# utiasDSL/gym-pybullet-drones

Hardware: AMD Instinct MI355X
Metric: env steps/sec (whole node), HoverAviary N=65536 drones @240Hz (higher is better)
Workload: dtype f32

## Files before the change

gym_pybullet_drones_amd/csrc/gpd_common.inc:

```
#pragma once
#include <hip/hip_runtime.h>
#include <rccl/rccl.h>
#include <dlfcn.h>

#include <cstdio>
#include <cstdlib>
#include <cstring>
#include <string>
#include <type_traits>

#include "gpd.h"

namespace {

#pragma clang fp contract(off)

#ifndef GPD_BLOCK
#define GPD_BLOCK 256
#endif
constexpr int kBlock = GPD_BLOCK;

template <auto V> using Const = std::integral_constant<decltype(V), V>;

}
// ... 88 lines not shown
    return (stride0 < 0 || stride1 < 0 || stride2 < 0) ? bad(GPD_EINVAL, "strides must be non-negative") : 0;
}
[[maybe_unused]] int check_ranges(Refuse bad, const GpdStepCfg* cfg) {
    if (cfg->act_type < GPD_ACT_RPM || cfg->act_type > GPD_ACT_DIRECT_RPM) return bad(GPD_EINVAL, "unknown act_type");
    return (cfg->task < GPD_TASK_NONE || cfg->task > GPD_TASK_MULTIHOVER) ? bad(GPD_EINVAL, "unknown task") : 0;
}
[[maybe_unused]] int check_positive(Refuse bad, const GpdStepCfg* cfg) {
    const bool ok = cfg->num_envs > 0 && cfg->drones_per_env > 0 && cfg->substeps > 0;
    return ok ? 0 : bad(GPD_EINVAL, "num_envs, drones_per_env and substeps must be positive");
}
[[maybe_unused]] int check_flags(Refuse bad, const GpdStepCfg* cfg) { return (cfg->physics_flags & ~31u) ? bad(GPD_EINVAL, "unknown physics flag") : 0; }
[[maybe_unused]] int check_extent(Refuse bad, int64_t N, int64_t ld, const char* pitch = "state.ld") {
    if (ld < N) return bad(GPD_EINVAL, pitch, " < num_envs*drones_per_env");
    return N > (1LL << 26) ? bad(GPD_ERANGE, "more than 2^26 drones per launch (32-bit byte offsets)") : 0;
}
[[maybe_unused]] int check_needs(Refuse bad, const GpdParams* params, const GpdState* state, const GpdStepCfg* cfg, const float* target_pos,
                                 const float* init_pose) {
    const bool pid = cfg->act_type == GPD_ACT_PID || cfg->act_type == GPD_ACT_VEL || cfg->act_type == GPD_ACT_ONE_D_PID;
    if (pid && state && !state->pid) return bad(GPD_EINVAL, "PID action type needs state.pid");
    if (pid && params->pid_kf <= 0.0f) return bad(GPD_ENOTSUP, "no DSLPID controller for this airframe (CF2X/CF2P only)");
    if ((cfg->physics_flags & GPD_PHYS_DRAG) && state && !state->last_rpm) return bad(GPD_EINVAL, "GPD_PHYS_DRAG needs state.last_rpm");
    if (cfg->task != GPD_TASK_NONE && !target_pos) return bad(GPD_EINVAL, "task needs target_pos");
    return (cfg->auto_reset && !init_pose) ? bad(GPD_EINVAL, "auto_reset needs init_pose") : 0;
}
[[maybe_unused]] void dummy_target(GpdStepCfg& c, const float*& target_pos, const float* readable) {
    if (c.task == GPD_TASK_NONE) { target_pos = readable; c.target_per_env = 0; }
}
template <class F>
auto with_ext_plant(bool ext, bool plant, F&& f) {
    if (plant) return ext ? f(Const<true>{}, Const<true>{}) : f(Const<false>{}, Const<true>{});
    return ext ? f(Const<true>{}, Const<false>{}) : f(Const<false>{}, Const<false>{});
}

struct Mat3 {
    float r00, r01, r02, r10, r11, r12, r20, r21, r22;
    float m22;
};

__device__ __forceinline__ float fast_rcp(float x) { return __builtin_amdgcn_rcpf(x); }
__device__ __forceinline__ float fast_sqrt(float x) { return __builtin_amdgcn_sqrtf(x); }
__device__ __forceinline__ float fast_rsq(float x) { return __builtin_amdgcn_rsqf(x); }
__device__ __forceinline__ float fast_exp(float x) { return __builtin_amdgcn_exp2f(x * 1.44269504088896340736f); }

typedef float fp2 __attribute__((ext_vector_type(2)));
__device__ __forceinline__ fp2 fma2(fp2 a, fp2 b, fp2 c) { return __builtin_elementwise_fma(a, b, c); }
__device__ __forceinline__ fp2 splat(float s) { return fp2{s, s}; }

__device__ __forceinline__ uint64_t lane_mask_opaque(bool p) {
    uint64_t m = __builtin_amdgcn_ballot_w64(p);
    asm volatile("" : "+s"(m));
    return m;
}
#define any_lane(p) __builtin_expect(lane_mask_opaque(p) != 0, 0)


__device__ __forceinline__ float atan2_poly(float y, float x) {
#pragma clang fp contract(off)
    const float ax = fabsf(x), ay = fabsf(y);
    const float mx = fmaxf(ax, ay), mn = fminf(ax, ay);
    float t = mn * fast_rcp(mx);
    t = (mx == 0.0f) ? 0.0f : t;
    const float u = t * t;
    float p = 2.766283504e-03f;
    p = fmaf(p, u, -1.573124913e-02f);
    p = fmaf(p, u, 4.213762361e-02f);
    p = fmaf(p, u, -7.456854827e-02f);
    p = fmaf(p, u, 1.061837064e-01f);
    p = fmaf(p, u, -1.419779779e-01f);
    p = fmaf(p, u, 1.999187203e-01f);
    p = fmaf(p, u, -3.333303671e-01f);
    p = fmaf(p, u, 9.999999818e-01f);
    p *= t;
    p = (ay > ax) ? (1.57079632679489661923f - p) : p;
    p = (x < 0.0f) ? (3.14159265358979323846f - p) : p;
    return copysignf(p, y);
}

__device__ __forceinline__ fp2 atan2_poly2(fp2 y, fp2 x) {
#pragma clang fp contract(off)
    const float ax0 = fabsf(x.x), ay0 = fabsf(y.x), ax1 = fabsf(x.y), ay1 = fabsf(y.y);
    const float mx0 = fmaxf(ax0, ay0), mn0 = fminf(ax0, ay0), mx1 = fmaxf(ax1, ay1), mn1 = fminf(ax1, ay1);
    fp2 t = fp2{mn0, mn1} * fp2{fast_rcp(mx0), fast_rcp(mx1)};
    t = fp2{(mx0 == 0.0f) ? 0.0f : t.x, (mx1 == 0.0f) ? 0.0f : t.y};
    const fp2 u = t * t;
    fp2 p = splat(2.766283504e-03f);
    p = fma2(p, u, splat(-1.573124913e-02f));
    p = fma2(p, u, splat(4.213762361e-02f));
    p = fma2(p, u, splat(-7.456854827e-02f));
    p = fma2(p, u, splat(1.061837064e-01f));
    p = fma2(p, u, splat(-1.419779779e-01f));
    p = fma2(p, u, splat(1.999187203e-01f));
    p = fma2(p, u, splat(-3.333303671e-01f));
    p = fma2(p, u, splat(9.999999818e-01f));
    p = p * t;
    float p0 = p.x, p1 = p.y;
    p0 = (ay0 > ax0) ? (1.57079632679489661923f - p0) : p0;
    p1 = (ay1 > ax1) ? (1.57079632679489661923f - p1) : p1;
    p0 = (x.x < 0.0f) ? (3.14159265358979323846f - p0) : p0;
    p1 = (x.y < 0.0f) ? (3.14159265358979323846f - p1) : p1;
    return fp2{copysignf(p0, y.x), copysignf(p1, y.y)};
}

__device__ __forceinline__ float asin_poly(float s) {
#pragma clang fp contract(off)
    return atan2_poly(s, fast_sqrt(fmaxf((1.0f - s) * (1.0f + s), 0.0f)));
}

__device__ __forceinline__ Mat3 quat_to_mat(float x, float y, float z, float w) {
    const float d = fmaf(x, x, fmaf(y, y, fmaf(z, z, w * w)));
    const float s = 2.0f * fast_rcp(d);
    const fp2 xys = fp2{x, y} * splat(s);
    const float xs = xys.x, ys = xys.y, zs = z * s;
    const fp2 wxy = splat(w) * xys;
    const float wx = wxy.x, wy = wxy.y, wz = w * zs;
    Mat3 R;
    R.r00 = 1.0f - fmaf(y, ys, z * zs); R.r01 = fmaf(x, ys, -wz);           R.r02 = fmaf(x, zs, wy);
    R.r10 = fmaf(x, ys, wz);            R.r11 = 1.0f - fmaf(x, xs, z * zs); R.r12 = fmaf(y, zs, -wx);
    R.m22 = fmaf(x, xs, y * ys);
    R.r20 = fmaf(x, zs, -wy);           R.r21 = fmaf(y, zs, wx);            R.r22 = 1.0f - R.m22;
    return R;
}

__device__ __forceinline__ void quat_to_rpy(float x, float y, float z, float w,
                                            float& roll, float& pitch, float& yaw) {
#pragma clang fp contract(off)
    const float sarg = -2.0f * fmaf(x, z, -(w * y));
    const float ww_zz = fmaf(w, w, z * z);
    const float xx_yy = fmaf(x, x, y * y);
    const float ww_yy = fmaf(w, w, -(y * y));
    const float xx_zz = fmaf(x, x, -(z * z));
    const fp2 ry = atan2_poly2(splat(2.0f) * fp2{fmaf(y, z, w * x), fmaf(x, y, w * z)}, fp2{ww_zz - xx_yy, ww_yy + xx_zz});
    roll = ry.x;
    pitch = asin_poly(fminf(fmaxf(sarg, -1.0f), 1.0f));
    yaw = ry.y;
    const bool gimbal = fabsf(sarg) >= 0.99999f;
    if (any_lane(gimbal)) {
        asm volatile("; gimbal lock: rare");
        if (gimbal) {
            const bool neg = sarg < 0.0f;
            roll = 0.0f;
            pitch = neg ? -1.57079632679489661923f : 1.57079632679489661923f;
            yaw = 2.0f * (neg ? atan2_poly(x, -y) : atan2_poly(-x, y));
        }
    }
}

__device__ __forceinline__ float clampf(float v, float lo, float hi) {
    return fminf(fmaxf(v, lo), hi);
}

struct Kin {
    float px, py, pz, qx, qy, qz, qw, vx, vy, vz, wx, wy, wz;
};

struct Pid {
    float ipx, ipy, ipz, lr, lp, ly, irx, iry, irz;
};

__device__ __forceinline__ void dslpid(const GpdParams& P, float dt, float inv_dt, const Kin& k, float roll, float pitch,
                                       float yaw, const Mat3& R, float tx, float ty, float tz, float tyaw,
                                       float tvx, float tvy, float tvz, float trr, float trp, float try_,
                                       Pid& s, float rpm[4], float pos_e[3], float* yaw_e) {
    const float epx = tx - k.px, epy = ty - k.py, epz = tz - k.pz;
    const float evx = tvx - k.vx, evy = tvy - k.vy, evz = tvz - k.vz;
    s.ipx = clampf(fmaf(epx, dt, s.ipx), -2.0f, 2.0f);
    s.ipy = clampf(fmaf(epy, dt, s.ipy), -2.0f, 2.0f);
    s.ipz = clampf(clampf(fmaf(epz, dt, s.ipz), -2.0f, 2.0f), -0.15f, 0.15f);
    const float fx = fmaf(P.d_for[0], evx, fmaf(P.i_for[0], s.ipx, P.p_for[0] * epx));
    const float fy = fmaf(P.d_for[1], evy, fmaf(P.i_for[1], s.ipy, P.p_for[1] * epy));
    const float fz = fmaf(P.d_for[2], evz, fmaf(P.i_for[2], s.ipz, P.p_for[2] * epz)) + P.pid_gravity;
    const float along = fmaxf(0.0f, fmaf(fz, R.r22, fmaf(fy, R.r12, fx * R.r02)));
    const float base_pwm = (fast_sqrt(along * P.pid_inv_4kf) - P.pwm2rpm_const) * P.inv_pwm2rpm_scale;
    const float fn = fast_rsq(fmaf(fz, fz, fmaf(fy, fy, fx * fx)));
    const float zbx = fx * fn, zby = fy * fn, zbz = fz * fn;
    float sy, cy;
    sincosf(tyaw, &sy, &cy);
    float ybx = -(zbz * sy);
    float yby = zbz * cy;
    float ybz = fmaf(zbx, sy, -(zby * cy));
    const float yn = fast_rsq(fmaf(ybz, ybz, fmaf(yby, yby, ybx * ybx)));
    ybx *= yn; yby *= yn; ybz *= yn;
    const float xbx = fmaf(yby, zbz, -(ybz * zby));
    const float xby = fmaf(ybz, zbx, -(ybx * zbz));
    const float xbz = fmaf(ybx, zby, -(yby * zbx));
    const float m21 = fmaf(zbz, R.r21, fmaf(zby, R.r11, zbx * R.r01)), m12 = fmaf(ybz, R.r22, fmaf(yby, R.r12, ybx * R.r02));
    const float m02 = fmaf(xbz, R.r22, fmaf(xby, R.r12, xbx * R.r02)), m20 = fmaf(zbz, R.r20, fmaf(zby, R.r10, zbx * R.r00));
    const float m10 = fmaf(ybz, R.r20, fmaf(yby, R.r10, ybx * R.r00)), m01 = fmaf(xbz, R.r21, fmaf(xby, R.r11, xbx * R.r01));
    const float erx = m21 - m12, ery = m02 - m20, erz = m10 - m01;
    const float ewx = fmaf(-(roll - s.lr), inv_dt, trr);
    const float ewy = fmaf(-(pitch - s.lp), inv_dt, trp);
    const float ewz = fmaf(-(yaw - s.ly), inv_dt, try_);
    s.lr = roll; s.lp = pitch; s.ly = yaw;
    s.irx = clampf(clampf(fmaf(-erx, dt, s.irx), -1500.0f, 1500.0f), -1.0f, 1.0f);
    s.iry = clampf(clampf(fmaf(-ery, dt, s.iry), -1500.0f, 1500.0f), -1.0f, 1.0f);
    s.irz = clampf(fmaf(-erz, dt, s.irz), -1500.0f, 1500.0f);
    const float t0 = clampf(fmaf(P.i_tor[0], s.irx, fmaf(P.d_tor[0], ewx, -(P.p_tor[0] * erx))), -3200.0f, 3200.0f);
    const float t1 = clampf(fmaf(P.i_tor[1], s.iry, fmaf(P.d_tor[1], ewy, -(P.p_tor[1] * ery))), -3200.0f, 3200.0f);
    const float t2 = clampf(fmaf(P.i_tor[2], s.irz, fmaf(P.d_tor[2], ewz, -(P.p_tor[2] * erz))), -3200.0f, 3200.0f);
#pragma unroll
    for (int m = 0; m < 4; ++m) {
        const float pwm = clampf(fmaf(P.mixer[3 * m + 2], t2, fmaf(P.mixer[3 * m + 1], t1, fmaf(P.mixer[3 * m], t0, base_pwm))),
                                 P.min_pwm, P.max_pwm);
        rpm[m] = fmaf(P.pwm2rpm_scale, pwm, P.pwm2rpm_const);
    }
    if (pos_e) { pos_e[0] = epx; pos_e[1] = epy; pos_e[2] = epz; }
    if (yaw_e) {
        *yaw_e = atan2_poly(-ybx, xbx) - yaw;
    }
}

__device__ __forceinline__ float thrust_dev(const GpdParams& P, float rpm) {
    return fmaf(P.KF * (rpm - P.hover_rpm), rpm + P.hover_rpm, P.hover_resid);
}
__device__ __forceinline__ float thrust_dev_norm(const GpdParams& P, float e) {
    return P.hover_thrust * (e * (2.0f + e));
}
__device__ __forceinline__ fp2 thrust_dev_norm2(const GpdParams& P, fp2 e) {
    return splat(P.hover_thrust) * (e * (splat(2.0f) + e));
}

struct PlantParams : GpdParams {
    float norm_thrust;
    float norm_gap;
};
__device__ __forceinline__ float thrust_dev_norm(const PlantParams& P, float e) {
    return P.norm_thrust * (e * (2.0f + e)) - P.norm_gap;
}
__device__ __forceinline__ fp2 thrust_dev_norm2(const PlantParams& P, fp2 e) {
    return splat(P.norm_thrust) * (e * (splat(2.0f) + e)) - splat(P.norm_gap);
}

template <bool EXT, bool AV = true>
__device__ __forceinline__ void substep(const GpdParams& P, float h, uint32_t flags, const float g[4],
                                        float drag_rpm_sum, float dw_force, Kin& k,
                                        float& avx, float& avy, float& avz) {
    const Mat3 R = quat_to_mat(k.qx, k.qy, k.qz, k.qw);
    float f0 = g[0], f1 = g[1], f2 = g[2], f3 = g[3];
    if (EXT && (flags & GPD_PHYS_GND)) {
        float e[4];
#pragma unroll
        for (int i = 0; i < 4; i += 2) {
            fp2 hz = fma2(splat(R.r21), fp2{P.prop_y[i], P.prop_y[i + 1]}, fma2(splat(R.r20), fp2{P.prop_x[i], P.prop_x[i + 1]}, splat(k.pz)));
            hz = fp2{fmaxf(hz.x, P.gnd_eff_h_clip), fmaxf(hz.y, P.gnd_eff_h_clip)};
            const fp2 ratio = splat(0.25f * P.prop_radius) * fp2{fast_rcp(hz.x), fast_rcp(hz.y)};
            const fp2 ei = ((splat(P.hover_thrust) + fp2{g[i], g[i + 1]}) * splat(P.gnd_eff_coeff)) * (ratio * ratio);
            e[i] = ei.x; e[i + 1] = ei.y;
        }
        const float sarg = -2.0f * fmaf(k.qx, k.qz, -(k.qw * k.qy));
        const float a = 2.0f * fmaf(k.qy, k.qz, k.qw * k.qx);
        const float b = fmaf(k.qw, k.qw, k.qz * k.qz) - fmaf(k.qx, k.qx, k.qy * k.qy);
        const bool on = (sarg > -0.99999f) && (sarg < 0.99999f) && (b > 0.0f || (a == 0.0f && b == 0.0f));
        if (on) { f0 += e[0]; f1 += e[1]; f2 += e[2]; f3 += e[3]; }
    }
    float dev = ((f0 + f1) + f2) + f3;
    if (EXT && (flags & GPD_PHYS_DW)) dev += dw_force;
    const float T = P.GRAVITY + dev;
    const fp2 Fxy = fp2{R.r02, R.r12} * splat(T);
    float Fx = Fxy.x, Fy = Fxy.y, Fz = fmaf(R.r22, dev, -(P.GRAVITY * R.m22));
    if (EXT && (flags & GPD_PHYS_DRAG)) {
        const float wsum = drag_rpm_sum * (6.28318530717958647692f / 60.0f);
        Fx = fmaf(-(P.drag_coeff[0] * k.vx), wsum, Fx);
        Fy = fmaf(-(P.drag_coeff[1] * k.vy), wsum, Fy);
        Fz = fmaf(-(P.drag_coeff[2] * k.vz), wsum, Fz);
    }
    if (EXT && (flags & GPD_PHYS_DAMP)) {
        const float vn = fast_sqrt(fmaf(k.vz, k.vz, fmaf(k.vy, k.vy, k.vx * k.vx)));
        const float ml = -(P.M * GPD_BULLET_DAMPING) * (1.0f + vn);
        Fx = fmaf(ml, k.vx, Fx); Fy = fmaf(ml, k.vy, Fy); Fz = fmaf(ml, k.vz, Fz);
    }
    const float kz = (P.drone_model == GPD_MODEL_RACE) ? -P.km_over_kf : P.km_over_kf;
    const float tz = kz * (((-g[0] + g[1]) - g[2]) + g[3]);
    const float arm = P.L * 0.70710678118654752440f;
    const float arm_x = (P.drone_model == GPD_MODEL_CF2X) ? -arm : arm;
    const float tx_x = (((f0 + f1) - f2) - f3) * arm_x, ty_x = (((-f0 + f1) + f2) - f3) * arm;
    const float tx_p = (f1 - f3) * P.L, ty_p = (-f0 + f2) * P.L;
    const uint32_t plus = (P.drone_model == GPD_MODEL_CF2P) ? 0xffffffffu : 0u;
    float tx = __uint_as_float((__float_as_uint(tx_p) & plus) | (__float_as_uint(tx_x) & ~plus));
    float ty = __uint_as_float((__float_as_uint(ty_p) & plus) | (__float_as_uint(ty_x) & ~plus));
    const fp2 jwxy = fp2{P.J[0], P.J[1]} * fp2{k.wx, k.wy};
    const float jwx = jwxy.x, jwy = jwxy.y, jwz = P.J[2] * k.wz;
    fp2 txy = fp2{tx, ty} - fp2{fmaf(k.wy, jwz, -(k.wz * jwy)), fmaf(k.wz, jwx, -(k.wx * jwz))};
    float tzz = tz - fmaf(k.wx, jwy, -(k.wy * jwx));
    if (EXT && (flags & GPD_PHYS_DAMP)) {
        const float wn = fast_sqrt(fmaf(k.wz, k.wz, fmaf(k.wy, k.wy, k.wx * k.wx)));
        const float da = -GPD_BULLET_DAMPING * (1.0f + wn);
        txy = fma2(jwxy, splat(da), txy);
        tzz = fmaf(jwz, da, tzz);
    }
    const fp2 hh = splat(h);
    const fp2 vxy = fma2(hh, fp2{Fx, Fy} * splat(P.inv_M), fp2{k.vx, k.vy});
    k.vx = vxy.x; k.vy = vxy.y; k.vz = fmaf(h, Fz * P.inv_M, k.vz);
    const fp2 wxy = fma2(hh, fp2{P.J_INV[0], P.J_INV[1]} * txy, fp2{k.wx, k.wy});
    k.wx = wxy.x; k.wy = wxy.y; k.wz = fmaf(h, P.J_INV[2] * tzz, k.wz);
    const fp2 pxy = fma2(hh, vxy, fp2{k.px, k.py});
    k.px = pxy.x; k.py = pxy.y; k.pz = fmaf(h, k.vz, k.pz);
    if (EXT && (flags & GPD_PHYS_GROUND)) {
        const bool hit = (k.pz < P.ground_z) | ((k.pz <= P.ground_z) & (k.vz < 0.0f));
        k.pz = hit ? P.ground_z : k.pz;
        k.vz = hit ? fmaxf(k.vz, 0.0f) : k.vz;
        k.vx = hit ? 0.0f : k.vx;
        k.vy = hit ? 0.0f : k.vy;
    }
    const float n2 = fmaf(k.wz, k.wz, fmaf(k.wy, k.wy, k.wx * k.wx));
    const float u = n2 * (0.25f * h * h);
    const fp2 uu = splat(u);
    const fp2 csp = fma2(fma2(fma2(fma2(fp2{2.412107309e-05f, 2.693749890e-06f}, uu, fp2{-1.388295778e-03f, -1.983586443e-04f}), uu,
                                  fp2{4.166645522e-02f, 8.333314057e-03f}), uu, fp2{-4.999999736e-01f, -1.666666643e-01f}), uu,
                        fp2{9.999999995e-01f, 1.0f});
    float cs = csp.x;
    float sc = csp.y * (0.5f * h);
    const bool tumbling = !(u <= 1.0f);
    if (any_lane(tumbling)) {
        asm volatile("; tumbling: rare");
        if (tumbling) {
            const float n = sqrtf(n2);
            float sn;
            sincosf(n * h * 0.5f, &sn, &cs);
            sc = sn / n;
        }
    }
    {
        const float lx = fmaf(k.wx, k.qw, fmaf(k.wz, k.qy, -(k.wy * k.qz)));
        const float ly = fmaf(k.wy, k.qw, fmaf(k.wx, k.qz, -(k.wz * k.qx)));
        const float lz = fmaf(k.wz, k.qw, fmaf(k.wy, k.qx, -(k.wx * k.qy)));
        const float lw = -fmaf(k.wz, k.qz, fmaf(k.wy, k.qy, k.wx * k.qx));
        const bool turn = n2 > 1e-16f;
        const fp2 nxy = fma2(splat(sc), fp2{lx, ly}, splat(cs) * fp2{k.qx, k.qy});
        const fp2 nzw = fma2(splat(sc), fp2{lz, lw}, splat(cs) * fp2{k.qz, k.qw});
        k.qx = turn ? nxy.x : k.qx; k.qy = turn ? nxy.y : k.qy;
        k.qz = turn ? nzw.x : k.qz; k.qw = turn ? nzw.y : k.qw;
    }
    if (AV) {
        const fp2 axy = fma2(fp2{R.r02, R.r12}, splat(k.wz), fma2(fp2{R.r01, R.r11}, splat(k.wy), fp2{R.r00, R.r10} * splat(k.wx)));
        avx = axy.x; avy = axy.y;
        avz = fmaf(R.r22, k.wz, fmaf(R.r21, k.wy, R.r20 * k.wx));
    }
}

__device__ __forceinline__ float ld_row(const float* __restrict__ base, int64_t ld, int r, uint32_t off4) {
    return *reinterpret_cast<const float*>(reinterpret_cast<const char*>(base + r * ld) + off4);
}
template <bool PLANT> using plant_t = std::conditional_t<PLANT, PlantParams, const GpdParams&>;
template <bool PLANT>
__device__ __forceinline__ plant_t<PLANT> plant_of(const GpdParams& P, const float* __restrict__ rows, int64_t ld, uint32_t off4) {
    if constexpr (PLANT) {
        PlantParams Q;
        static_cast<GpdParams&>(Q) = P;
        Q.M = ld_row(rows, ld, GPD_PLANT_M, off4);
        Q.inv_M = ld_row(rows, ld, GPD_PLANT_INV_M, off4);
        Q.KF = ld_row(rows, ld, GPD_PLANT_KF, off4);
        Q.GRAVITY = ld_row(rows, ld, GPD_PLANT_GRAVITY, off4);
        Q.J[0] = ld_row(rows, ld, GPD_PLANT_J, off4);
        Q.J[1] = ld_row(rows, ld, GPD_PLANT_J + 1, off4);
        Q.J[2] = ld_row(rows, ld, GPD_PLANT_J + 2, off4);
        Q.J_INV[0] = ld_row(rows, ld, GPD_PLANT_J_INV, off4);
        Q.J_INV[1] = ld_row(rows, ld, GPD_PLANT_J_INV + 1, off4);
        Q.J_INV[2] = ld_row(rows, ld, GPD_PLANT_J_INV + 2, off4);
        Q.km_over_kf = ld_row(rows, ld, GPD_PLANT_KM_OVER_KF, off4);
        Q.gnd_eff_coeff = ld_row(rows, ld, GPD_PLANT_GND_EFF, off4);
        Q.drag_coeff[0] = ld_row(rows, ld, GPD_PLANT_DRAG, off4);
        Q.drag_coeff[1] = ld_row(rows, ld, GPD_PLANT_DRAG + 1, off4);
        Q.drag_coeff[2] = ld_row(rows, ld, GPD_PLANT_DRAG + 2, off4);
        Q.hover_thrust = ld_row(rows, ld, GPD_PLANT_HOVER_THRUST, off4);
        Q.hover_resid = ld_row(rows, ld, GPD_PLANT_HOVER_RESID, off4);
        Q.norm_thrust = ld_row(rows, ld, GPD_PLANT_NORM_THRUST, off4);
        Q.norm_gap = ld_row(rows, ld, GPD_PLANT_NORM_GAP, off4);
        return Q;
    } else {
        (void)rows; (void)ld; (void)off4;
        return P;
    }
}
template <bool PLANT>
__device__ __forceinline__ void plant_live(const plant_t<PLANT>& Q) {
    if constexpr (PLANT)
        asm volatile("" :: "v"(Q.M), "v"(Q.inv_M), "v"(Q.KF), "v"(Q.GRAVITY), "v"(Q.J[0]), "v"(Q.J[1]), "v"(Q.J[2]), "v"(Q.J_INV[0]),
                           "v"(Q.J_INV[1]), "v"(Q.J_INV[2]), "v"(Q.km_over_kf), "v"(Q.gnd_eff_coeff), "v"(Q.drag_coeff[0]),
                           "v"(Q.drag_coeff[1]), "v"(Q.drag_coeff[2]), "v"(Q.hover_thrust), "v"(Q.hover_resid), "v"(Q.norm_thrust),
                           "v"(Q.norm_gap) : "memory");
    else
        (void)Q;
}

template <bool NT = false>
__device__ __forceinline__ void st_row(float* __restrict__ base, int64_t ld, int r, uint32_t off4, float v) {
    float* p = reinterpret_cast<float*>(reinterpret_cast<char*>(base + r * ld) + off4);
    if (NT) __builtin_nontemporal_store(v, p);
    else *p = v;
}

__device__ __forceinline__ const float4* kin_P(const float* kin, int64_t ld) { (void)ld; return reinterpret_cast<const float4*>(kin); }
__device__ __forceinline__ const float4* kin_Q(const float* kin, int64_t ld) { return reinterpret_cast<const float4*>(kin + 4 * ld); }
__device__ __forceinline__ const float4* kin_V(const float* kin, int64_t ld) { return reinterpret_cast<const float4*>(kin + 8 * ld); }
__device__ __forceinline__ float4* kin_P(float* kin, int64_t ld) { (void)ld; return reinterpret_cast<float4*>(kin); }
__device__ __forceinline__ float4* kin_Q(float* kin, int64_t ld) { return reinterpret_cast<float4*>(kin + 4 * ld); }
__device__ __forceinline__ float4* kin_V(float* kin, int64_t ld) { return reinterpret_cast<float4*>(kin + 8 * ld); }

__device__ __forceinline__ void store_obs12(float* __restrict__ obs, uint32_t n, float px, float py, float pz,
                                            float roll, float pitch, float yaw, float vx, float vy, float vz,
                                            float ax, float ay, float az) {
    float4* o = reinterpret_cast<float4*>(reinterpret_cast<char*>(obs) + n * 48u);
    o[0] = make_float4(px, py, pz, roll);
    o[1] = make_float4(pitch, yaw, vx, vy);
    o[2] = make_float4(vz, ax, ay, az);
}

__device__ __forceinline__ void wg_barrier() {
    __builtin_amdgcn_s_waitcnt(0xC07F);
    __builtin_amdgcn_s_barrier();
}

struct Lane {
    uint32_t n;
    uint32_t env;
    int tid;
    int le, d;
    int base;
    bool active;
    bool shfl;
};

struct Carry {
    Kin k;
    Pid s;
    float l0, l1, l2, l3;
    int counter;
    float dw_in;
    float roll, pitch, yaw;
};

struct StepOut {
    float o[12];
    float to[12];
    float rew;
    bool term, trunc, reset;
};

template <bool PID, int AW, int ACT, class PP>
__device__ __forceinline__ void map_action(const PP& P, const GpdStepCfg& C, const float4 act, Carry& c,
                                           float rpm[4], float g[4]) {
    const Kin& k = c.k;
    const int act_type = ACT >= 0 ? ACT : C.act_type;
    rpm[0] = rpm[1] = rpm[2] = rpm[3] = 0.0f;
    if (!PID) {
        if (AW == 1) {
            const float e = 0.05f * act.x;
            rpm[0] = rpm[1] = rpm[2] = rpm[3] = fmaf(P.hover_rpm, e, P.hover_rpm);
            g[0] = g[1] = g[2] = g[3] = thrust_dev_norm(P, e);
        } else if (act_type == GPD_ACT_RPM) {
            const fp2 e01 = splat(0.05f) * fp2{act.x, act.y}, e23 = splat(0.05f) * fp2{act.z, act.w};
            const fp2 r01 = fma2(splat(P.hover_rpm), e01, splat(P.hover_rpm)), r23 = fma2(splat(P.hover_rpm), e23, splat(P.hover_rpm));
            const fp2 g01 = thrust_dev_norm2(P, e01), g23 = thrust_dev_norm2(P, e23);
            rpm[0] = r01.x; rpm[1] = r01.y; rpm[2] = r23.x; rpm[3] = r23.y;
            g[0] = g01.x; g[1] = g01.y; g[2] = g23.x; g[3] = g23.y;
        } else {
            const bool clip = act_type == GPD_ACT_RAW_RPM;
            const float lo = clip ? 0.0f : -3.0e38f, hi = clip ? P.max_rpm : 3.0e38f;
            rpm[0] = clampf(act.x, lo, hi); rpm[1] = clampf(act.y, lo, hi);
            rpm[2] = clampf(act.z, lo, hi); rpm[3] = clampf(act.w, lo, hi);
#pragma unroll
            for (int i = 0; i < 4; ++i) g[i] = thrust_dev(P, rpm[i]);
        }
    } else {
        float tx = k.px, ty = k.py, tz = k.pz, tyaw = 0.0f, tvx = 0.0f, tvy = 0.0f, tvz = 0.0f;
        if (AW == 3) {
            const float dx = act.x - k.px, dy = act.y - k.py, dz = act.z - k.pz;
            const float d2 = fmaf(dz, dz, fmaf(dy, dy, dx * dx));
            if (fast_sqrt(d2) <= 1.0f) { tx = act.x; ty = act.y; tz = act.z; }
            else { const float id = fast_rsq(d2); tx = fmaf(dx, id, k.px); ty = fmaf(dy, id, k.py); tz = fmaf(dz, id, k.pz); }
        } else if (AW == 4) {
            const float nn2 = fmaf(act.z, act.z, fmaf(act.y, act.y, act.x * act.x));
            const float sp = P.speed_limit * fabsf(act.w);
            if (nn2 != 0.0f) { const float in = fast_rsq(nn2); tvx = sp * (act.x * in); tvy = sp * (act.y * in); tvz = sp * (act.z * in); }
            tyaw = c.yaw;
        } else {
            tz = fmaf(0.1f, act.x, k.pz);
        }
        const Mat3 R = quat_to_mat(k.qx, k.qy, k.qz, k.qw);
        dslpid(P, C.ctrl_dt, C.inv_ctrl_dt, k, c.roll, c.pitch, c.yaw, R, tx, ty, tz, tyaw, tvx, tvy, tvz, 0.0f, 0.0f, 0.0f,
               c.s, rpm, nullptr, nullptr);
#pragma unroll
        for (int i = 0; i < 4; ++i) g[i] = thrust_dev(P, rpm[i]);
    }
}

__device__ __forceinline__ void task_single(const GpdStepCfg& C, float px, float py, float pz, float roll, float pitch,
                                            int counter, float tgx, float tgy, float tgz, float& rew, bool& term,
                                            bool& trunc) {
    const fp2 exy = fp2{tgx, tgy} - fp2{px, py};
    const float ex = exy.x, ey = exy.y, ez = tgz - pz;
    const float my_dist = fast_sqrt(fmaf(ez, ez, fmaf(ey, ey, ex * ex)));
    const float d2 = my_dist * my_dist;
    rew = fmaxf(0.0f, fmaf(-d2, d2, 2.0f));
    const bool my_out = (fabsf(px) > C.xy_bound) | (fabsf(py) > C.xy_bound) | (pz > C.z_bound) |
                        (fabsf(roll) > C.tilt_bound) | (fabsf(pitch) > C.tilt_bound);
    term = my_dist < C.term_dist;
    trunc = my_out | (counter > C.trunc_counter);
}

__device__ __forceinline__ float pair_mate(float v) {
    return __int_as_float(__builtin_amdgcn_mov_dpp(__float_as_int(v), 0xB1, 0xf, 0xf, true));
}

template <bool PID, bool EXT, bool MULTI, int AW, int ACT = -1, bool S1 = false, class PP = GpdParams>
__device__ __forceinline__ void env_step(const PP& P, const GpdStepCfg& C, const uint32_t flags, const int D,
                                         const Lane& L, const float4 act, const float tgx, const float tgy,
                                         const float tgz, const bool ip_regs, const float* __restrict__ ipose,
                                         const float ip0, const float ip1, const float ip2, const float ip3,
                                         const float ip4, const float ip5, const float ip6, float* sh_pos,
                                         float* sh_red, Carry& c, StepOut& out, const float* irpy = nullptr) {
    Kin& k = c.k;
    float rpm[4], g[4];
    map_action<PID, AW, ACT>(P, C, act, c, rpm, g);

    const float cur_sum = ((rpm[0] + rpm[1]) + rpm[2]) + rpm[3];
    float drag_sum = (EXT && (flags & GPD_PHYS_DRAG)) ? ((c.l0 + c.l1) + c.l2) + c.l3 : cur_sum;
    float avx = 0.0f, avy = 0.0f, avz = 0.0f;
    if (S1 && !(EXT && MULTI)) {
        substep<EXT>(P, C.pyb_dt, flags, g, drag_sum, EXT ? c.dw_in : 0.0f, k, avx, avy, avz);
    } else if (!MULTI) {
        const float dw = EXT ? c.dw_in : 0.0f;
        int left = C.substeps;
        for (; left > 2; left -= 2) {
            substep<EXT, false>(P, C.pyb_dt, flags, g, drag_sum, dw, k, avx, avy, avz);
            substep<EXT, false>(P, C.pyb_dt, flags, g, cur_sum, dw, k, avx, avy, avz);
            drag_sum = cur_sum;
        }
        if (left == 2) {
            substep<EXT, false>(P, C.pyb_dt, flags, g, drag_sum, dw, k, avx, avy, avz);
            drag_sum = cur_sum;
        }
        substep<EXT, true>(P, C.pyb_dt, flags, g, drag_sum, dw, k, avx, avy, avz);
    } else
    for (int ss = 0, nsub = S1 ? 1 : C.substeps; ss < nsub; ++ss) {
        float dw = (EXT && !MULTI) ? c.dw_in : 0.0f;
        if (EXT && MULTI && (flags & GPD_PHYS_DW)) {
            auto wake_of = [&](float xj, float yj, float zj) {
                const float dz = zj - k.pz;
                const float ddx = xj - k.px, ddy = yj - k.py;
                const float dxy2 = fmaf(ddy, ddy, ddx * ddx);
                const float ratio = (0.25f * P.prop_radius) * fast_rcp(dz);
                const float alpha = P.dw_coeff[0] * (ratio * ratio);
                const float beta = fmaf(P.dw_coeff[1], dz, P.dw_coeff[2]);
                const float ib = fast_rcp(beta);
                const float pushed = dw - alpha * fast_exp(-0.5f * (dxy2 * (ib * ib)));
                dw = ((dz > 0.0f) & (dxy2 < 100.0f)) ? pushed : dw;
            };
            float dwc0 = P.dw_coeff[0], dwc1 = P.dw_coeff[1], dwc2 = P.dw_coeff[2];
            asm volatile("" : "+s"(dwc0), "+s"(dwc1), "+s"(dwc2));
            const fp2 mx = splat(k.px), my = splat(k.py), mz = splat(k.pz), qr = splat(0.25f * P.prop_radius);
            auto two_mates = [&](fp2 xj, fp2 yj, fp2 zj) {
                const fp2 dz = zj - mz, ddx = xj - mx, ddy = yj - my;
                const fp2 dxy2 = fma2(ddy, ddy, ddx * ddx);
                const fp2 ratio = qr * fp2{fast_rcp(dz.x), fast_rcp(dz.y)};
                const fp2 alpha = splat(dwc0) * (ratio * ratio);
                const fp2 beta = fma2(splat(dwc1), dz, splat(dwc2));
                const fp2 ib = fp2{fast_rcp(beta.x), fast_rcp(beta.y)};
                const fp2 arg = (splat(-0.5f) * (dxy2 * (ib * ib))) * splat(1.44269504088896340736f);
                const fp2 push = alpha * fp2{__builtin_amdgcn_exp2f(arg.x), __builtin_amdgcn_exp2f(arg.y)};
                const float p0 = dw - push.x;
                dw = ((dz.x > 0.0f) & (dxy2.x < 100.0f)) ? p0 : dw;
                const float p1 = dw - push.y;
                dw = ((dz.y > 0.0f) & (dxy2.y < 100.0f)) ? p1 : dw;
            };
            const float* const sx = sh_pos + L.base;
            auto pair_at = [&](int j) {
                two_mates(fp2{sx[j], sx[j + 1]}, fp2{sx[kBlock + j], sx[kBlock + j + 1]}, fp2{sx[2 * kBlock + j], sx[2 * kBlock + j + 1]});
            };
            if (L.shfl) {
                if (D == 2) {
// ... 226 lines not shown
```

gym_pybullet_drones_amd/csrc/step_rollout.hip:

```cpp
#include "gpd_common.inc"
#include "policy_kernel.inc"
#include <iterator>
#include <utility>

namespace {

template <bool PID, bool EXT, bool MULTI, int AW, int ACT, bool S1, int DC = 0, int FL = -1, bool HI = false, bool PLANT = false>
__global__ __launch_bounds__(kBlock) void gpd_step_kernel(
    float* __restrict__ hot_kin, const float* __restrict__ action, int32_t* __restrict__ hot_counter,
    const float* __restrict__ target_pos, const int32_t* __restrict__ hot_slot, const uint32_t hot_ld, const int32_t hot_num_envs,
    const int32_t hot_lanes_per_wave, const int32_t hot_target_per_env,
    const GpdParams P, const GpdState S_, const GpdStepCfg C_, const float* __restrict__ init_pose, float* __restrict__ obs12,
    float* __restrict__ reward, uint8_t* __restrict__ terminated, uint8_t* __restrict__ truncated,
    float* __restrict__ term_obs12, uint32_t* __restrict__ done_flag, const uint32_t done_seq, const float* __restrict__ plant) {
    const GpdState S{hot_kin, S_.last_rpm, S_.pid, hot_counter, static_cast<int64_t>(hot_ld), S_.dw_force, S_.act_ring, S_.ring_pos, S_.hist_len, 0, S_.bad};
    const GpdStepCfg C{hot_num_envs, C_.drones_per_env, C_.act_type, C_.substeps, C_.physics_flags, C_.pyb_dt, C_.ctrl_dt, C_.inv_ctrl_dt,
                       hot_lanes_per_wave, C_.task, C_.xy_bound, C_.z_bound, C_.tilt_bound, C_.term_dist, C_.trunc_counter, hot_target_per_env,
                       C_.init_per_env, C_.auto_reset};
    const int D = MULTI ? (DC ? DC : C.drones_per_env) : 1;
    const int tid = threadIdx.x;
    const uint32_t N = static_cast<uint32_t>(C.num_envs) * static_cast<uint32_t>(D);
    const int LW = MULTI ? 64 : C.lanes_per_wave;
    const int lanes = MULTI ? (kBlock / D) * D : (kBlock / 64) * LW;
    const uint32_t n_raw = MULTI ? blockIdx.x * lanes + tid : (blockIdx.x * (kBlock / 64) + (tid >> 6)) * LW + (tid & 63);
// ... 273 lines not shown
    };
    if (!PID) {
        float4 a0 = fetch(0), a1, a2;
        __builtin_amdgcn_sched_barrier(0);
        a1 = fetch(1);
        __builtin_amdgcn_sched_barrier(0);
        for (int t = 0; t < K; t += 3) {
            a2 = fetch(t + 2);
            do_step(t, a0);
            if (t + 1 >= K) break;
            a0 = fetch(t + 3);
            do_step(t + 1, a1);
            if (t + 2 >= K) break;
            a1 = fetch(t + 4);
            do_step(t + 2, a2);
        }
    } else {
        float4 act = fetch(0);
        for (int t = 0; t < K; ++t) {
            const float4 act_next = fetch(t + 1);
            do_step(t, act);
            act = act_next;
        }
    }
    if (L.active) store_carry<PID>(S, L, c);
}

template <bool NT_OBS = true>
struct RollOut {
    char* og_prev; char* og; char* rg; uint8_t* tg; uint8_t* ug;
    int64_t obs_step, env_step;
    uint32_t g0, g1, g2, e4, e1;
    float4* mine; const char* lsrc;
    f4v pend[3];
    __device__ __forceinline__ RollOut(float* obs12, float* reward, uint8_t* terminated, uint8_t* truncated, const Span& T,
                                       const uint32_t goff[3], uint32_t eoff4, uint32_t env, float* row, const char* lsrc_)
        : og_prev(reinterpret_cast<char*>(obs12)), og(reinterpret_cast<char*>(obs12)), rg(reinterpret_cast<char*>(reward)),
          tg(terminated), ug(truncated), obs_step(T.obs_stride * 4), env_step(T.env_stride), g0(goff[0]), g1(goff[1]),
          g2(goff[2]), e4(eoff4), e1(env), mine(reinterpret_cast<float4*>(row)), lsrc(lsrc_) {
        pend[0] = pend[1] = pend[2] = f4v{0, 0, 0, 0};
    }
    __device__ __forceinline__ void bursts(char* base) {
        asm volatile("" : "+v"(g0), "+v"(g1), "+v"(g2));
        if (NT_OBS) {
            __builtin_nontemporal_store(pend[0], reinterpret_cast<f4v*>(base + g0));
            __builtin_nontemporal_store(pend[1], reinterpret_cast<f4v*>(base + g1));
            __builtin_nontemporal_store(pend[2], reinterpret_cast<f4v*>(base + g2));
        } else {
            *reinterpret_cast<f4v*>(base + g0) = pend[0];
            *reinterpret_cast<f4v*>(base + g1) = pend[1];
            *reinterpret_cast<f4v*>(base + g2) = pend[2];
        }
    }
    __device__ __forceinline__ void emit(const StepOut& out, bool advance) {
        if (advance) { og_prev = og; og += obs_step; rg += env_step * 4; tg += env_step; ug += env_step; }
        bursts(og_prev);
        mine[0] = make_float4(out.o[0], out.o[1], out.o[2], out.o[3]);
        mine[1] = make_float4(out.o[4], out.o[5], out.o[6], out.o[7]);
        mine[2] = make_float4(out.o[8], out.o[9], out.o[10], out.o[11]);
        __builtin_amdgcn_wave_barrier();
#pragma unroll
        for (int j = 0; j < 3; ++j) {
            const float4 v = *reinterpret_cast<const float4*>(lsrc + j * 1024);
            pend[j] = f4v{v.x, v.y, v.z, v.w};
        }
        __builtin_amdgcn_wave_barrier();
        asm volatile("" : "+v"(e4), "+v"(e1));
        __builtin_nontemporal_store(out.rew, reinterpret_cast<float*>(rg + e4));
        __builtin_nontemporal_store(static_cast<uint8_t>(out.term ? 1 : 0), tg + e1);
        __builtin_nontemporal_store(static_cast<uint8_t>(out.trunc ? 1 : 0), ug + e1);
    }
    __device__ __forceinline__ void flush() { bursts(og); }
};

template <bool PID, bool EXT, int AW, int ACT, bool S1, bool MULTI, bool NT_OBS = true, bool RING = false, int DC = 0, int FL = -1, bool HI = false,
          bool PLANT = false>
__global__ __launch_bounds__(kBlock) void gpd_rollout1_kernel(
    float* __restrict__ hot_kin, const float* __restrict__ action, int32_t* __restrict__ hot_counter, const float* __restrict__ target_pos,
    const float* __restrict__ init_pose, const uint32_t hot_ld, const int32_t hot_num_envs, const int32_t hot_num_steps, const uint32_t hot_bits,
    const GpdParams P, const GpdState S_, const GpdStepCfg C_, const Span T_, float* __restrict__ obs12,
    float* __restrict__ reward, uint8_t* __restrict__ terminated, uint8_t* __restrict__ truncated,
    float* __restrict__ term_obs12, const float* __restrict__ plant) {
    const GpdState S{hot_kin, S_.last_rpm, S_.pid, hot_counter, static_cast<int64_t>(hot_ld), S_.dw_force, S_.act_ring, S_.ring_pos, S_.hist_len, 0, S_.bad};
    const GpdStepCfg C{hot_num_envs, C_.drones_per_env, C_.act_type, C_.substeps, C_.physics_flags, C_.pyb_dt, C_.ctrl_dt, C_.inv_ctrl_dt,
                       C_.lanes_per_wave, C_.task, C_.xy_bound, C_.z_bound, C_.tilt_bound, C_.term_dist, C_.trunc_counter,
                       static_cast<int32_t>((hot_bits >> 2) & 1u), static_cast<int32_t>((hot_bits >> 1) & 1u), static_cast<int32_t>(hot_bits & 1u)};
    const Span T{hot_num_steps, T_.action_stride, T_.obs_stride, T_.env_stride, T_.ring};
    const int tid = threadIdx.x;
    uint32_t bid = blockIdx.x;
    if (hot_bits & 8u) { const uint32_t per = gridDim.x >> 3; bid = (blockIdx.x & 7u) * per + (blockIdx.x >> 3); }
    const int D = MULTI ? (DC ? DC : C.drones_per_env) : 1;
    const uint32_t N = static_cast<uint32_t>(C.num_envs) * static_cast<uint32_t>(D);
    const int K = T.num_steps;
    const uint32_t flags = EXT ? (FL >= 0 ? (static_cast<uint32_t>(FL) | (HI ? C.physics_flags & ~7u : 0u)) : C.physics_flags) : 0u;
    const int wave0 = tid & ~63, lane = tid & 63;
    const int W = MULTI ? (64 / D) * D : 64;
    const uint32_t block_base = bid * static_cast<uint32_t>(4 * W);
    const uint32_t n0 = block_base + static_cast<uint32_t>((tid >> 6) * W);
    const uint32_t rows = n0 < N ? ((N - n0 < static_cast<uint32_t>(W)) ? N - n0 : static_cast<uint32_t>(W)) : 0u;
    const uint32_t first = rows ? n0 : block_base;
    auto drone_of = [&](uint32_t r) {
        if (!MULTI) return r < rows ? n0 + r : block_base;
        const uint32_t rw = static_cast<uint32_t>(W);
        return r < rows ? n0 + r : first + (r < rw ? r - (r / static_cast<uint32_t>(D)) * static_cast<uint32_t>(D) : r - rw);
    };
    Lane L;
    L.tid = tid; L.shfl = MULTI;
    L.le = MULTI ? tid / D : tid;
    L.active = static_cast<uint32_t>(lane) < rows;
    L.n = drone_of(static_cast<uint32_t>(lane));
    L.d = MULTI ? static_cast<int>(L.n % static_cast<uint32_t>(D)) : 0;
    L.base = MULTI ? wave0 + (lane < W ? (lane / D) * D : 0) : tid;
    L.env = MULTI ? L.n / static_cast<uint32_t>(D) : L.n;

    __shared__ __attribute__((aligned(16))) float sh_rows[kBlock * 12];
    __shared__ __attribute__((aligned(16))) float sh_pos[MULTI ? 4 * kBlock : 4];
    __shared__ __attribute__((aligned(16))) float sh_red[MULTI ? 4 * kBlock : 4];

    uint32_t goff[3];
    const char* lsrc = reinterpret_cast<const char*>(sh_rows + wave0 * 12) + lane * 16;
#pragma unroll
    for (int j = 0; j < 3; ++j) {
        const uint32_t cidx = static_cast<uint32_t>(j * 64 + lane), r = cidx / 3u, part = cidx - 3u * r;
        goff[j] = drone_of(r) * 48u + part * 16u;
    }
    const uint32_t eoff4 = L.env * 4u;

    Carry c;
    float tgx, tgy, tgz, ip[7];
    auto fetch = [&](int step) { return load_action<AW, true>(action + (step < K ? step : K - 1) * T.action_stride, L.n); };
    const float* ipose = reinterpret_cast<const float*>(reinterpret_cast<const char*>(init_pose) +
                                                        (C.init_per_env ? L.n * 28u : static_cast<uint32_t>(L.d) * 28u));
    load_carry<PID, EXT>(S, C, flags, L, target_pos, C.auto_reset ? ipose : S.kin, c, tgx, tgy, tgz, ip);
    int ring_q = 0;
    if constexpr (RING) {
        ring_q = S.ring_pos[L.env];
        GPD_DBG(ring_q >= 0 && ring_q < S.hist_len, GPD_DBG_RING_POS, ring_q); ring_q = GPD_DBG_CLAMP(ring_q, 0, S.hist_len - 1);
    }
    asm volatile("" :: "v"(c.k.px), "v"(c.k.py), "v"(c.k.pz), "v"(c.k.qx), "v"(c.k.qy), "v"(c.k.qz), "v"(c.k.qw), "v"(c.k.vx),
                       "v"(c.k.vy), "v"(c.k.vz), "v"(c.k.wx), "v"(c.k.wy), "v"(c.k.wz), "v"(tgx), "v"(tgy), "v"(tgz),
                       "v"(c.counter), "v"(ip[0]), "v"(ip[1]), "v"(ip[2]), "v"(ip[3]), "v"(ip[4]), "v"(ip[5]), "v"(ip[6])
                 : "memory");
    if constexpr (RING) asm volatile("" :: "v"(ring_q) : "memory");
    plant_t<PLANT> Q = plant_of<PLANT>(P, plant, S.ld, L.n * 4u);
    plant_live<PLANT>(Q);
    __builtin_amdgcn_s_waitcnt(0x0F70);
    __builtin_amdgcn_s_barrier();
    c.roll = c.pitch = c.yaw = 0.0f;
    if (PID) quat_to_rpy(c.k.qx, c.k.qy, c.k.qz, c.k.qw, c.roll, c.pitch, c.yaw);

    (void)term_obs12;
    RollOut<NT_OBS> ro(obs12, reward, terminated, truncated, T, goff, eoff4, L.env, sh_rows + tid * 12, lsrc);
    float irpy[3] = {0.0f, 0.0f, 0.0f};
    if (C.auto_reset) quat_to_rpy(ip[3], ip[4], ip[5], ip[6], irpy[0], irpy[1], irpy[2]);
    auto do_step = [&](const int t, const float4 act) {
        StepOut out;
        env_step<PID, EXT, MULTI, AW, ACT, S1>(Q, C, flags, D, L, act, tgx, tgy, tgz, true, ipose, ip[0], ip[1], ip[2], ip[3],
                                               ip[4], ip[5], ip[6], sh_pos, sh_red, c, out, irpy);
        ro.emit(out, t > 0);
        if constexpr (RING) {
            const size_t slot = static_cast<size_t>(N) * AW;
            float* r0 = S.act_ring + static_cast<size_t>(ring_q) * slot + static_cast<size_t>(L.n) * AW;
            float* r1 = r0 + static_cast<size_t>(S.hist_len) * slot;
            if (AW == 4) { *reinterpret_cast<float4*>(r0) = act; *reinterpret_cast<float4*>(r1) = act; }
            else { r0[0] = act.x; r1[0] = act.x; if (AW == 3) { r0[1] = act.y; r0[2] = act.z; r1[1] = act.y; r1[2] = act.z; } }
            ring_q = ring_q + 1 == S.hist_len ? 0 : ring_q + 1;
        }
    };
    if (!PID) {
        float4 a0 = fetch(0), a1 = fetch(1), a2 = fetch(2);
        asm volatile("" :: "v"(a0.x), "v"(a0.y), "v"(a0.z), "v"(a0.w), "v"(a1.x), "v"(a1.y), "v"(a1.z), "v"(a1.w), "v"(a2.x),
                           "v"(a2.y), "v"(a2.z), "v"(a2.w) : "memory");
        __builtin_amdgcn_s_waitcnt(0x0F70);
        for (int t = 0; t < K; t += 3) {
            const float4 b0 = fetch(t + 3), b1 = fetch(t + 4), b2 = fetch(t + 5);
            do_step(t, a0);
            if (t + 1 >= K) break;
            do_step(t + 1, a1);
            if (t + 2 >= K) break;
            do_step(t + 2, a2);
            asm volatile("" :: "v"(b0.x), "v"(b0.y), "v"(b0.z), "v"(b0.w), "v"(b1.x), "v"(b1.y), "v"(b1.z), "v"(b1.w),
                               "v"(b2.x), "v"(b2.y), "v"(b2.z), "v"(b2.w) : "memory");
            a0 = b0; a1 = b1; a2 = b2;
        }
    } else {
        float4 a = fetch(0);
        asm volatile("" :: "v"(a.x), "v"(a.y), "v"(a.z), "v"(a.w) : "memory");
        __builtin_amdgcn_s_waitcnt(0x0F70);
        for (int t = 0; t < K; ++t) {
            const float4 b = fetch(t + 1);
            do_step(t, a);
            asm volatile("" :: "v"(b.x), "v"(b.y), "v"(b.z), "v"(b.w) : "memory");
            a = b;
        }
    }
    ro.flush();
    if (L.active) store_carry<PID>(S, L, c);
    if constexpr (RING) { if (L.active && L.d == 0) S.ring_pos[L.env] = ring_q; }
}

template <int ACT> constexpr bool kSizedAct = ACT != GPD_ACT_RAW_RPM && ACT != GPD_ACT_DIRECT_RPM;

struct Variant {
    bool multi, s1;
    int dc, fl;
    bool hi;
    constexpr bool sized() const { return dc != 0 || fl >= 0 || (multi && s1); }
    bool fits(const GpdStepCfg& C) const {
        return multi == (C.drones_per_env > 1) && (!s1 || C.substeps == 1) && (dc == 0 || dc == C.drones_per_env) &&
               (fl < 0 || ((C.physics_flags & 7u) == static_cast<uint32_t>(fl) && (hi || (C.physics_flags & ~7u) == 0u)));
    }
};
// ... 282 lines not shown
```

Measured before the change: 79.98 billion.

## Merge rare tumbling, gimbal and reset branches into one deferred wave check

For the single-drone, one-substep, non-PID path, the kernel now defers the rare tumbling quaternion fix and the gimbal-lock RPY fix. It runs one combined ballot across tumbling, gimbal and episode-end masks, and the fixup path recomputes the quaternion, RPY and task reward only on lanes that hit a rare case. Several divergent branches per step collapse into a single uniform check, and term/trunc flags are carried as words to simplify the stores. The cost is duplicated task evaluation code and extra live registers for the deferred state, which may raise register pressure.

```diff
diff --git a/gym_pybullet_drones_amd/csrc/gpd_common.inc b/gym_pybullet_drones_amd/csrc/gpd_common.inc
--- a/gym_pybullet_drones_amd/csrc/gpd_common.inc
+++ b/gym_pybullet_drones_amd/csrc/gpd_common.inc
@@ -164,6 +164,8 @@
     return m;
 }
 #define any_lane(p) __builtin_expect(lane_mask_opaque(p) != 0, 0)
+__device__ __forceinline__ uint64_t mask_opaque(uint64_t m) { asm volatile("" : "+s"(m)); return m; }
+#define any_mask(m) __builtin_expect(mask_opaque(m) != 0, 0)
 
 
 __device__ __forceinline__ float atan2_poly(float y, float x) {
@@ -233,8 +235,9 @@
     return R;
 }
 
+template <bool DEFER = false>
 __device__ __forceinline__ void quat_to_rpy(float x, float y, float z, float w,
-                                            float& roll, float& pitch, float& yaw) {
+                                            float& roll, float& pitch, float& yaw, bool* gimbal_out = nullptr) {
 #pragma clang fp contract(off)
     const float sarg = -2.0f * fmaf(x, z, -(w * y));
     const float ww_zz = fmaf(w, w, z * z);
@@ -246,6 +249,7 @@
     pitch = asin_poly(fminf(fmaxf(sarg, -1.0f), 1.0f));
     yaw = ry.y;
     const bool gimbal = fabsf(sarg) >= 0.99999f;
+    if constexpr (DEFER) { *gimbal_out = gimbal; return; }
     if (any_lane(gimbal)) {
         asm volatile("; gimbal lock: rare");
         if (gimbal) {
@@ -342,10 +346,16 @@
     return splat(P.norm_thrust) * (e * (splat(2.0f) + e)) - splat(P.norm_gap);
 }
 
-template <bool EXT, bool AV = true>
+struct RareFix {
+    float qx, qy, qz, qw;
+    float n2;
+    bool tumbling;
+    bool gimbal;
+};
+template <bool EXT, bool AV = true, int DEFER = 0>
 __device__ __forceinline__ void substep(const GpdParams& P, float h, uint32_t flags, const float g[4],
                                         float drag_rpm_sum, float dw_force, Kin& k,
-                                        float& avx, float& avy, float& avz) {
+                                        float& avx, float& avy, float& avz, RareFix* rare = nullptr) {
     const Mat3 R = quat_to_mat(k.qx, k.qy, k.qz, k.qw);
     float f0 = g[0], f1 = g[1], f2 = g[2], f3 = g[3];
     if (EXT && (flags & GPD_PHYS_GND)) {
@@ -422,6 +432,10 @@
     float cs = csp.x;
     float sc = csp.y * (0.5f * h);
     const bool tumbling = !(u <= 1.0f);
+    if constexpr (DEFER) {
+        rare->qx = k.qx; rare->qy = k.qy; rare->qz = k.qz; rare->qw = k.qw; rare->n2 = n2; rare->tumbling = tumbling;
+        if constexpr (DEFER == 2) __builtin_amdgcn_sched_barrier(0);
+    } else
     if (any_lane(tumbling)) {
         asm volatile("; tumbling: rare");
         if (tumbling) {
@@ -447,6 +461,25 @@
         avx = axy.x; avy = axy.y;
         avz = fmaf(R.r22, k.wz, fmaf(R.r21, k.wy, R.r20 * k.wx));
     }
+}
+
+__device__ __forceinline__ void rare_fixup(float h, const RareFix& f, Kin& k, float& roll, float& pitch, float& yaw) {
+    if (f.tumbling) {
+        const float n = sqrtf(f.n2);
+        float sn, cs;
+        sincosf(n * h * 0.5f, &sn, &cs);
+        const float sc = sn / n;
+        const float lx = fmaf(k.wx, f.qw, fmaf(k.wz, f.qy, -(k.wy * f.qz)));
+        const float ly = fmaf(k.wy, f.qw, fmaf(k.wx, f.qz, -(k.wz * f.qx)));
+        const float lz = fmaf(k.wz, f.qw, fmaf(k.wy, f.qx, -(k.wx * f.qy)));
+        const float lw = -fmaf(k.wz, f.qz, fmaf(k.wy, f.qy, k.wx * f.qx));
+        const bool turn = f.n2 > 1e-16f;
+        const fp2 nxy = fma2(splat(sc), fp2{lx, ly}, splat(cs) * fp2{f.qx, f.qy});
+        const fp2 nzw = fma2(splat(sc), fp2{lz, lw}, splat(cs) * fp2{f.qz, f.qw});
+        k.qx = turn ? nxy.x : f.qx; k.qy = turn ? nxy.y : f.qy;
+        k.qz = turn ? nzw.x : f.qz; k.qw = turn ? nzw.y : f.qw;
+    }
+    quat_to_rpy(k.qx, k.qy, k.qz, k.qw, roll, pitch, yaw);
 }
 
 __device__ __forceinline__ float ld_row(const float* __restrict__ base, int64_t ld, int r, uint32_t off4) {
@@ -546,6 +579,7 @@
     float to[12];
     float rew;
     bool term, trunc, reset;
+    uint32_t term_w, trunc_w;
 };
 
 template <bool PID, int AW, int ACT, class PP>
@@ -614,7 +648,7 @@
     return __int_as_float(__builtin_amdgcn_mov_dpp(__float_as_int(v), 0xB1, 0xf, 0xf, true));
 }
 
-template <bool PID, bool EXT, bool MULTI, int AW, int ACT = -1, bool S1 = false, class PP = GpdParams>
+template <bool PID, bool EXT, bool MULTI, int AW, int ACT = -1, bool S1 = false, int FUSED = 0, class PP = GpdParams>
 __device__ __forceinline__ void env_step(const PP& P, const GpdStepCfg& C, const uint32_t flags, const int D,
                                          const Lane& L, const float4 act, const float tgx, const float tgy,
                                          const float tgz, const bool ip_regs, const float* __restrict__ ipose,
@@ -628,6 +662,62 @@
     const float cur_sum = ((rpm[0] + rpm[1]) + rpm[2]) + rpm[3];
     float drag_sum = (EXT && (flags & GPD_PHYS_DRAG)) ? ((c.l0 + c.l1) + c.l2) + c.l3 : cur_sum;
     float avx = 0.0f, avy = 0.0f, avz = 0.0f;
+    if constexpr (FUSED) {
+        static_assert(S1 && !MULTI, "the fused step is the single-drone, one-sub-step form");
+        RareFix fx;
+        substep<EXT, true, FUSED>(P, C.pyb_dt, flags, g, drag_sum, EXT ? c.dw_in : 0.0f, k, avx, avy, avz, &fx);
+        quat_to_rpy<true>(k.qx, k.qy, k.qz, k.qw, c.roll, c.pitch, c.yaw, &fx.gimbal);
+        if constexpr (FUSED == 2) __builtin_amdgcn_sched_barrier(0);
+        const bool has_task = C.task != GPD_TASK_NONE;
+        const uint32_t auto_u = C.auto_reset != 0 ? 1u : 0u;
+        float r;
+        bool te, tr;
+        task_single(C, k.px, k.py, k.pz, c.roll, c.pitch, c.counter, tgx, tgy, tgz, r, te, tr);
+        float rew = has_task ? r : -1.0f;
+        uint32_t term_u = (has_task & te) ? 1u : 0u, trunc_u = (has_task & tr) ? 1u : 0u;
+        asm volatile("" : "+v"(term_u), "+v"(trunc_u));
+        __builtin_assume(term_u <= 1u); __builtin_assume(trunc_u <= 1u);
+        uint32_t reset_u = (term_u | trunc_u) & auto_u;
+        asm volatile("" : "+v"(reset_u));
+        const bool do_reset = reset_u != 0u;
+        int counter = do_reset ? 0 : c.counter + C.substeps;
+        asm volatile("" : "+v"(counter));
+        c.l0 = rpm[0]; c.l1 = rpm[1]; c.l2 = rpm[2]; c.l3 = rpm[3];
+        auto episode_end = [&]() {
+            out.to[0] = k.px; out.to[1] = k.py; out.to[2] = k.pz; out.to[3] = c.roll; out.to[4] = c.pitch; out.to[5] = c.yaw;
+            out.to[6] = k.vx; out.to[7] = k.vy; out.to[8] = k.vz; out.to[9] = avx; out.to[10] = avy; out.to[11] = avz;
+            if (ip_regs) k = Kin{ip0, ip1, ip2, ip3, ip4, ip5, ip6, 0, 0, 0, 0, 0, 0};
+            else k = Kin{ipose[0], ipose[1], ipose[2], ipose[3], ipose[4], ipose[5], ipose[6], 0, 0, 0, 0, 0, 0};
+            if (irpy) { c.roll = irpy[0]; c.pitch = irpy[1]; c.yaw = irpy[2]; }
+            else quat_to_rpy(k.qx, k.qy, k.qz, k.qw, c.roll, c.pitch, c.yaw);
+            avx = avy = avz = 0.0f;
+            c.l0 = c.l1 = c.l2 = c.l3 = 0.0f;
+        };
+        const bool redo = fx.tumbling | fx.gimbal;
+        const uint64_t rare = __builtin_amdgcn_ballot_w64(fx.tumbling) | __builtin_amdgcn_ballot_w64(fx.gimbal) | __builtin_amdgcn_ballot_w64(do_reset);
+        if (any_mask(rare)) {
+            asm volatile("; tumbling, gimbal lock or episode end: rare");
+            if (any_lane(redo)) {
+                asm volatile("; tumbling or gimbal lock");
+                if (redo) rare_fixup(C.pyb_dt, fx, k, c.roll, c.pitch, c.yaw);
+                float r2;
+                bool te2, tr2;
+                task_single(C, k.px, k.py, k.pz, c.roll, c.pitch, c.counter, tgx, tgy, tgz, r2, te2, tr2);
+                rew = has_task ? r2 : -1.0f;
+                term_u = (has_task & te2) ? 1u : 0u; trunc_u = (has_task & tr2) ? 1u : 0u;
+                reset_u = (term_u | trunc_u) & auto_u;
+                counter = reset_u != 0u ? 0 : c.counter + C.substeps;
+            }
+            if (reset_u != 0u) episode_end();
+        }
+        __builtin_assume(term_u <= 1u); __builtin_assume(trunc_u <= 1u);
+        c.counter = counter;
+        out.rew = rew; out.term = term_u != 0u; out.trunc = trunc_u != 0u; out.reset = reset_u != 0u;
+        out.term_w = term_u; out.trunc_w = trunc_u;
+        out.o[0] = k.px; out.o[1] = k.py; out.o[2] = k.pz; out.o[3] = c.roll; out.o[4] = c.pitch; out.o[5] = c.yaw;
+        out.o[6] = k.vx; out.o[7] = k.vy; out.o[8] = k.vz; out.o[9] = avx; out.o[10] = avy; out.o[11] = avz;
+        return;
+    }
     if (S1 && !(EXT && MULTI)) {
         substep<EXT>(P, C.pyb_dt, flags, g, drag_sum, EXT ? c.dw_in : 0.0f, k, avx, avy, avz);
     } else if (!MULTI) {
diff --git a/gym_pybullet_drones_amd/csrc/step_rollout.hip b/gym_pybullet_drones_amd/csrc/step_rollout.hip
--- a/gym_pybullet_drones_amd/csrc/step_rollout.hip
+++ b/gym_pybullet_drones_amd/csrc/step_rollout.hip
@@ -349,6 +349,7 @@
             *reinterpret_cast<f4v*>(base + g2) = pend[2];
         }
     }
+    template <bool WORDS = false>
     __device__ __forceinline__ void emit(const StepOut& out, bool advance) {
         if (advance) { og_prev = og; og += obs_step; rg += env_step * 4; tg += env_step; ug += env_step; }
         bursts(og_prev);
@@ -364,8 +365,8 @@
         __builtin_amdgcn_wave_barrier();
         asm volatile("" : "+v"(e4), "+v"(e1));
         __builtin_nontemporal_store(out.rew, reinterpret_cast<float*>(rg + e4));
-        __builtin_nontemporal_store(static_cast<uint8_t>(out.term ? 1 : 0), tg + e1);
-        __builtin_nontemporal_store(static_cast<uint8_t>(out.trunc ? 1 : 0), ug + e1);
+        __builtin_nontemporal_store(WORDS ? static_cast<uint8_t>(out.term_w) : static_cast<uint8_t>(out.term ? 1 : 0), tg + e1);
+        __builtin_nontemporal_store(WORDS ? static_cast<uint8_t>(out.trunc_w) : static_cast<uint8_t>(out.trunc ? 1 : 0), ug + e1);
     }
     __device__ __forceinline__ void flush() { bursts(og); }
 };
@@ -450,11 +451,12 @@
     RollOut<NT_OBS> ro(obs12, reward, terminated, truncated, T, goff, eoff4, L.env, sh_rows + tid * 12, lsrc);
     float irpy[3] = {0.0f, 0.0f, 0.0f};
     if (C.auto_reset) quat_to_rpy(ip[3], ip[4], ip[5], ip[6], irpy[0], irpy[1], irpy[2]);
+    constexpr int kFused = (!PID && !EXT && !MULTI && S1 && !PLANT) ? (NT_OBS ? 2 : 1) : 0;
     auto do_step = [&](const int t, const float4 act) {
         StepOut out;
-        env_step<PID, EXT, MULTI, AW, ACT, S1>(Q, C, flags, D, L, act, tgx, tgy, tgz, true, ipose, ip[0], ip[1], ip[2], ip[3],
-                                               ip[4], ip[5], ip[6], sh_pos, sh_red, c, out, irpy);
-        ro.emit(out, t > 0);
+        env_step<PID, EXT, MULTI, AW, ACT, S1, kFused>(Q, C, flags, D, L, act, tgx, tgy, tgz, true, ipose, ip[0], ip[1], ip[2], ip[3],
+                                                       ip[4], ip[5], ip[6], sh_pos, sh_red, c, out, irpy);
+        ro.template emit<kFused != 0>(out, t > 0);
         if constexpr (RING) {
             const size_t slot = static_cast<size_t>(N) * AW;
             float* r0 = S.act_ring + static_cast<size_t>(ring_q) * slot + static_cast<size_t>(L.n) * AW;
```

After: 77.27 billion. 0.966x the previous value.
